# merijn-23/magr-ray-tracer

Measured on AMD Instinct MI355X. Metric: Mrays/sec + extend-kernel HBM GB/s, sponza 1080p 256spp, higher is better.
Workload: dtype f32

## Files before the change

include/rt355.h:

```cpp
#ifndef RT355_H
#define RT355_H
#include "rt355_types.h"

#ifdef __cplusplus
extern "C" {
#endif

#define RT_OK            0
#define RT_E_INVALID    (-1)
#define RT_E_DEVICE     (-2)
#define RT_E_NOMEM      (-3)
#define RT_E_UNSUPPORTED (-4)

#define RT_SHADING_SIMPLE       0
#define RT_SHADING_NEE          1
#define RT_SAMPLING_HEMISPHERE  0
#define RT_SAMPLING_COSINE      1
#define RT_ACCEL_BVH2           0
#define RT_ACCEL_BVH4           1

typedef struct RtCtx RtCtx;

typedef struct RtConfig {
    int32_t width, height;
// ... 12 lines not shown

#define RT_BUILTINS_DEFAULT    0
#define RT_BUILTINS_IEEE       1
#define RT_BUILTINS_REFERENCE  2

typedef struct RtCounters {
    uint64_t extend_rays, extend_tlas_visits, extend_inst_visits, extend_node_visits, extend_prim_tests;
    uint64_t connect_rays, connect_tlas_visits, connect_inst_visits, connect_node_visits, connect_prim_tests;
    uint64_t primary_rays;
    uint64_t shadow_rays;
    uint64_t frames;
    uint64_t extend_node_issues, extend_leaf_issues, connect_node_issues, connect_leaf_issues;
    uint64_t extend_loop_node_events, extend_loop_leaf_events, connect_loop_node_events, connect_loop_leaf_events;
} RtCounters;

typedef struct RtStageTimes {
    double  generate_ms, extend_ms, shade_ms, compact_ms, connect_ms, accumulate_ms;
    int64_t generate_launches, extend_launches, shade_launches, compact_launches, connect_launches, accumulate_launches;
} RtStageTimes;

typedef struct RtKernelInfo {
    int32_t layout;
    int32_t persist, persist4;
    int32_t stack_entries;
    int32_t persist_grid, persist_grid_connect, shade_grid;
    int32_t n_blas;
} RtKernelInfo;

const char* rt_last_error(void);
int rt_device_count(void);
int rt_kernel_info(RtCtx* ctx, RtKernelInfo* out);
int rt_builtins(RtCtx* ctx);
int rt_top_levels(RtCtx* ctx, int32_t* extend, int32_t* connect);

int rt_create(const RtConfig* cfg, RtCtx** out);
int rt_destroy(RtCtx* ctx);

int rt_upload_scene(RtCtx* ctx,
                    const RtPrimitive* prims, int32_t nPrims,
                    const RtMaterial* mats, int32_t nMats,
                    const RtFloat4* textures, int32_t nTexels,
                    const uint32_t* lights, int32_t nLights,
                    const void* bvhNodes, int32_t nNodes,
                    const uint32_t* primIdx, int32_t nIdx,
                    const RtTLASNode* tlas, int32_t nTlas,
                    const RtBVHInstance* blas, int32_t nBlas);

int rt_upload_scene_bvh2(RtCtx* ctx,
                         const RtPrimitive* prims, int32_t nPrims, const RtMaterial* mats, int32_t nMats,
                         const RtFloat4* textures, int32_t nTexels, const uint32_t* lights, int32_t nLights,
                         const RtBVHNode2* bvhNodes, int32_t nNodes, const uint32_t* primIdx, int32_t nIdx,
                         const RtTLASNode* tlas, int32_t nTlas, const RtBVHInstance* blas, int32_t nBlas);

int rt_validate_scene(int32_t accel,
                      const RtPrimitive* prims, int32_t nPrims, const RtMaterial* mats, int32_t nMats,
                      const RtFloat4* textures, int32_t nTexels, const uint32_t* lights, int32_t nLights,
                      const void* bvhNodes, int32_t nNodes, const uint32_t* primIdx, int32_t nIdx,
                      const RtTLASNode* tlas, int32_t nTlas, const RtBVHInstance* blas, int32_t nBlas);

int rt_share_scene(RtCtx* ctx, RtCtx* from);

int rt_build_bvh2(int32_t device, const RtBuildOptions* opts, const RtPrimitive* prims, int32_t nPrims, int32_t first, int32_t count,
                  uint32_t nodeBase, uint32_t idxBase, RtBVHNode2* nodes, int32_t nodeCap, int32_t* nNodes, uint32_t* primIdx,
                  RtBuildStats* stats);
int rt_build_bvh2_sah(int32_t device, const RtPrimitive* prims, int32_t nPrims, int32_t first, int32_t count, uint32_t nodeBase,
                      uint32_t idxBase, RtBVHNode2* nodes, int32_t nodeCap, int32_t* nNodes, uint32_t* primIdx, RtBuildStats* stats);
// ... 141 lines not shown
```

magr_ray_tracer_amd/_lib.py:

```python
import ctypes as C
import os

import numpy as np

_PKG = os.path.dirname(os.path.abspath(__file__))

f4 = np.dtype((np.float32, 4))
Ray = np.dtype([("O", f4), ("D", f4), ("rD", f4), ("N", f4), ("I", f4), ("intensity", f4), ("t", "<f4"),
                ("primIdx", "<i4"), ("bounces", "<i4"), ("pixelIdx", "<i4"), ("inside", "u1"), ("lastSpecular", "u1"),
                ("_pad0", "u1", 2), ("u", "<f4"), ("v", "<f4"), ("_pad1", "<u4")], align=False)
ShadowRay = np.dtype([("I", f4), ("L", f4), ("Nl", f4), ("intensity", f4), ("BRDF", f4), ("lightIdx", "<i4"),
                      ("pixelIdx", "<i4"), ("dotNL", "<f4"), ("dist", "<f4")])
Material = np.dtype([("color", f4), ("absorption", f4), ("specular", "<f4"), ("n1", "<f4"), ("n2", "<f4"),
                     ("isDielectric", "u1"), ("_pad0", "u1", 3), ("texIdx", "<i4"), ("texW", "<i4"), ("texH", "<i4"),
                     ("isLight", "u1"), ("_pad1", "u1", 3), ("emittance", f4)])
Primitive = np.dtype([("v0", f4), ("v1", f4), ("v2", f4), ("N", f4), ("centroid", f4), ("uv0", "<f4", 2), ("uv1", "<f4", 2),
                      ("uv2", "<f4", 2), ("_padt", "<f4", 2), ("objType", "<i4"), ("matIdx", "<i4"), ("area", "<f4"),
                      ("_pad", "<u4")])
Camera = np.dtype([("type", "<i4"), ("fov", "<f4"), ("aperture", "<f4"), ("focalLength", "<f4"), ("forward", f4),
                   ("right", f4), ("up", f4), ("origin", f4), ("horizontal", f4), ("vertical", f4), ("topLeft", f4)])
Settings = np.dtype([("numPrimitives", "<i4"), ("numLights", "<i4"), ("tracerType", "<i4"), ("frames", "<i4"),
                     ("antiAliasing", "<i4"), ("numInRays", "<i4"), ("numOutRays", "<i4"), ("shadowRays", "<i4"),
                     ("renderBVH", "<i4"), ("focalLength", "<f4")])
BVHNode2 = np.dtype([("aabbMin", f4), ("aabbMax", f4), ("first", "<u4"), ("count", "<u4"), ("_pad", "<u4", 2)])
# ... 33 lines not shown
SAMPLING_HEMISPHERE, SAMPLING_COSINE = 0, 1
ACCEL_BVH2, ACCEL_BVH4 = 0, 1
PRIM_SPHERE, PRIM_PLANE, PRIM_TRIANGLE = 0, 1, 2
MATH_EXP, MATH_SIN, MATH_COS, MATH_ACOS, MATH_ATAN, MATH_F2I, MATH_ATAN2, MATH_SPHERE_TEXEL, MATH_NORMALIZE4, MATH_LENGTH4 = range(10)
MATH_WORDS = {MATH_EXP: (1, 1), MATH_SIN: (1, 1), MATH_COS: (1, 1), MATH_ACOS: (1, 1), MATH_ATAN: (1, 1), MATH_F2I: (1, 1),
              MATH_ATAN2: (2, 1), MATH_SPHERE_TEXEL: (6, 2), MATH_NORMALIZE4: (4, 4), MATH_LENGTH4: (4, 1)}
MATH_SWEEP_BLOCK_BITS = 20
MAX_BOUNCES = 7
BUILTINS_DEFAULT, BUILTINS_IEEE, BUILTINS_REFERENCE = 0, 1, 2
BUILTINS = {None: BUILTINS_DEFAULT, "ieee": BUILTINS_IEEE, "reference": BUILTINS_REFERENCE}


def builtins_value(name):
    try:
        return BUILTINS[name]
    except (KeyError, TypeError):
        raise ValueError(f"builtins must be None, 'ieee' or 'reference', not {name!r}") from None


RT_OK, RT_E_INVALID, RT_E_DEVICE, RT_E_NOMEM, RT_E_UNSUPPORTED = 0, -1, -2, -3, -4
SCENE_ARRAYS = {"prims": 0, "bvh": 1, "tlas": 2, "instances": 3, "pairs": 4, "triRecs": 5, "shadeRecs": 6, "lightRecs": 7,
                "tlasPairs": 8, "tlasPairsP": 9, "instRecs": 10}
SCENE_ARRAYS_BVH4 = {"quads": 11, "rootEntry": 12, "bvh2Kept": 13}
UpdateStats = np.dtype([("gpu_ms", "<f8"), ("prims", "<i4"), ("nodes", "<i4"), ("tlas_nodes", "<i4"), ("tlas_depth", "<i4"),
                        ("reconfigured", "<i4"), ("reserved", "<i4", 3)])
assert UpdateStats.itemsize == 40
REBUILD_SAH, REBUILD_LBVH, REBUILD_SBVH = 0, 1, 2
RebuildStats = np.dtype([(n, "<f8") for n in ("gpu_ms", "wall_ms", "stage_ms", "build_ms", "derive_ms", "tlas_ms", "commit_ms")] +
                        [(n, "<i4") for n in ("prims", "blas_built", "nodes", "n_idx", "max_depth", "tlas_nodes", "tlas_depth", "reconfigured")] +
                        [("spatial_splits", "<i4"), ("prims_clipped", "<i4")])
assert RebuildStats.itemsize == 96

DEVICE_SYMBOLS = [
    "rt_last_error", "rt_device_count", "rt_kernel_info", "rt_builtins", "rt_top_levels", "rt_create", "rt_destroy", "rt_upload_scene", "rt_share_scene", "rt_set_seeds", "rt_seed_default",
    "rt_get_seeds", "rt_bind_accum", "rt_accum_device_ptr", "rt_stream", "rt_reset", "rt_render", "rt_synchronize", "rt_focus",
    "rt_read_accum", "rt_write_accum", "rt_postproc", "rt_read_counters", "rt_reset_counters", "rt_read_stage_times", "rt_reset_stage_times", "rt_set_profile",
    "rt_stage_begin_frame", "rt_stage_generate", "rt_stage_extend", "rt_stage_shade", "rt_stage_connect",
    "rt_debug_get_rays", "rt_debug_set_rays", "rt_debug_get_shadow", "rt_debug_enable_steps", "rt_debug_get_steps", "rt_debug_math",
    "rt_debug_math_sweep", "rt_debug_math_mode", "rt_debug_math_sweep_mode", "rt_validate_scene", "rt_build_bvh2", "rt_build_bvh2_sah", "rt_debug_sah_phases", "rt_build_bvh2_sbvh", "rt_debug_sbvh_phases", "rt_update_scene", "rt_group_update_scene", "rt_debug_get_scene_array",
    "rt_rebuild_scene", "rt_group_rebuild_scene", "rt_blas_ranges", "rt_debug_rebuild_allocations",
    "rt_build_bvh4", "rt_upload_scene_bvh2", "rt_group_upload_scene_bvh2",
    "rt_group_create", "rt_group_destroy", "rt_group_lanes", "rt_group_concurrency", "rt_group_lane", "rt_group_frames", "rt_group_upload_scene", "rt_group_share_scene",
    "rt_group_seed", "rt_group_reset", "rt_group_render", "rt_group_synchronize", "rt_group_sum", "rt_group_read_accum", "rt_group_focus",
    "rt_group_postproc"]
HOST_SYMBOLS = [
    "rth_last_error", "rth_scene_create", "rth_scene_destroy", "rth_add_material", "rth_add_texture", "rth_load_texture", "rth_add_sphere",
    "rth_add_plane", "rth_add_triangle", "rth_add_quad", "rth_add_triangles", "rth_build_blas", "rth_build_bvh4",
    "rth_build_tlas", "rth_bvh4_from_nodes", "rth_set_instance_transform", "rth_primitives", "rth_materials", "rth_textures", "rth_lights",
    "rth_bvh2_nodes", "rth_bvh4_nodes", "rth_prim_idx", "rth_tlas_nodes", "rth_blas_nodes", "rth_bvh_stats", "rth_camera",
    "rth_renderer_create", "rth_renderer_destroy", "rth_renderer_init", "rth_renderer_set_camera", "rth_renderer_tick",
    "rth_renderer_read", "rth_renderer_camera", "rth_seed_stream", "rth_load_model", "rth_save_png",
    "rth_set_build_threads", "rth_renderer_save_frame", "rth_renderer_camera_move", "rth_renderer_camera_mouse", "rth_renderer_camera_zoom", "rth_renderer_frames", "rth_renderer_set_lanes", "rth_renderer_set_builtins", "rth_renderer_builtins",
    "rth_build_blas_lbvh", "rth_build_bvh2_lbvh", "rth_lbvh_stats", "rth_set_primitives", "rth_refit",
    "rth_build_blas_sah_gpu", "rth_build_bvh2_sah", "rth_build_blas_sbvh_gpu", "rth_build_bvh2_sbvh", "rth_rebuild", "rth_blas_ranges",
    "rth_build_bvh4_gpu", "rth_build_bvh4_levels"]

_dev = None
_host = None


class NativeLibraryMissing(RuntimeError):
    pass


def _load(name, local=False):
    path = os.path.join(_PKG, name)
    if not os.path.exists(path):
        raise NativeLibraryMissing(
            f"{path} is missing: build it with `python -m magr_ray_tracer_amd.build` (hipcc, gfx950). "
            "The hot path has no Python/CPU fallback.")
    return C.CDLL(path, mode=C.RTLD_LOCAL if local else C.RTLD_GLOBAL)


_variants = {}


def device_lib(variant=None):
    global _dev
    if variant:
        if variant not in _variants:
            keep, _dev = _dev, None
            try:
                _variants[variant] = _bind_device(_load(f"librt355_{variant}.so", local=True))
            finally:
                _dev = keep
        return _variants[variant]
    if _dev is None:
        _dev = _bind_device(_load("librt355.so"))
    return _dev


def _bind_device(lib):
    if True:
        vp, i32, i64 = C.c_void_p, C.c_int32, C.c_int64
        lib.rt_last_error.restype = C.c_char_p
        lib.rt_create.argtypes = [vp, C.POINTER(vp)]
        lib.rt_kernel_info.argtypes = [vp, vp]
        lib.rt_builtins.argtypes = [vp]
        lib.rt_top_levels.argtypes = [vp, C.POINTER(i32), C.POINTER(i32)]
        lib.rt_destroy.argtypes = [vp]
        lib.rt_upload_scene.argtypes = [vp, vp, i32, vp, i32, vp, i32, vp, i32, vp, i32, vp, i32, vp, i32, vp, i32]
        lib.rt_upload_scene_bvh2.argtypes = lib.rt_upload_scene.argtypes
        lib.rt_group_upload_scene_bvh2.argtypes = lib.rt_upload_scene.argtypes
        lib.rt_build_bvh4.argtypes = [i32, vp, i32, i32, vp, i32, vp, vp]
        lib.rt_share_scene.argtypes = [vp, vp]
        lib.rt_set_seeds.argtypes = [vp, vp, i64]
        lib.rt_seed_default.argtypes = [vp]
        lib.rt_get_seeds.argtypes = [vp, vp, i64]
        lib.rt_bind_accum.argtypes = [vp, vp]
        lib.rt_accum_device_ptr.argtypes = [vp]
        lib.rt_accum_device_ptr.restype = vp
        lib.rt_stream.argtypes = [vp]
        lib.rt_stream.restype = vp
        lib.rt_reset.argtypes = [vp]
        lib.rt_render.argtypes = [vp, vp, vp, i32]
        lib.rt_synchronize.argtypes = [vp]
        lib.rt_focus.argtypes = [vp, i32, i32, vp, C.POINTER(C.c_float)]
        lib.rt_read_accum.argtypes = [vp, vp]
        lib.rt_read_counters.argtypes = [vp, vp]
        lib.rt_write_accum.argtypes = [vp, vp]
        lib.rt_postproc.argtypes = [vp, i32, C.c_float, C.c_float, C.c_float, vp, vp]
        lib.rt_reset_counters.argtypes = [vp]
        lib.rt_read_stage_times.argtypes = [vp, vp]
        lib.rt_reset_stage_times.argtypes = [vp]
        lib.rt_set_profile.argtypes = [vp, i32]
        lib.rt_stage_begin_frame.argtypes = [vp]
        lib.rt_stage_generate.argtypes = [vp, vp, vp]
        lib.rt_stage_extend.argtypes = [vp, i32, i32]
        lib.rt_stage_shade.argtypes = [vp, i32]
        lib.rt_stage_connect.argtypes = [vp, i32, i32]
        lib.rt_debug_get_rays.argtypes = [vp, i32, vp, i32, C.POINTER(i32)]
        lib.rt_debug_set_rays.argtypes = [vp, i32, vp, i32]
# ... 120 lines not shown
```

magr_ray_tracer_amd/csrc/rt355.hip:

```cpp
#include <hip/hip_runtime.h>
#include <hip/hip_ext.h>
#include <algorithm>
#include <chrono>
#include <cstdio>
#include <cmath>
#include <cstdlib>
#include <cstring>
#include <memory>
#include <atomic>
#include <string>
#include <vector>
#include "../../include/rt355.h"
#include "rt355_kernels.h"
#include "scene_dev.h"

using namespace rt355dev;
using namespace scenedev;

static constexpr int kAdmitAnySgpr = 6, kAdmit96Sgpr = 7;
static constexpr int kTopLevelsExtend = 6, kTopLevelsConnect = 6;
static constexpr int kFitSeven = 22, kBackupWords = 10, kSpillCap = kFitSeven - kBackupWords;
static thread_local std::string g_err;
int rt355_set_error(int code, const char* msg) { g_err = msg; return code; }

// ... 76 lines not shown
static bool spill_trav(const RtCtx* c) { return c->trav == TRAV_TLAS_SPILL || c->trav == TRAV_BVH4_TLAS_SPILL; }
static bool bvh4_tlas_trav(const RtCtx* c) { return c->trav == TRAV_BVH4_TLAS || c->trav == TRAV_BVH4_TLAS_SPILL; }
static bool tlas_trav(const RtCtx* c) { return c->trav == TRAV_TLAS || c->trav == TRAV_TLAS_SPILL || bvh4_tlas_trav(c); }

extern "C" const char* rt_last_error(void) { return g_err.c_str(); }
extern "C" int rt_device_count(void) { int n = 0; if (hipGetDeviceCount(&n) != hipSuccess) return 0; return n; }
static int sync_scene_config(RtCtx* ctx);
extern "C" int rt_builtins(RtCtx* ctx)
{
    if (!ctx) return fail(RT_E_INVALID, "rt_builtins: null context");
    return ctx->cfg.builtins;
}
extern "C" int rt_kernel_info(RtCtx* ctx, RtKernelInfo* out)
{
    if (!ctx || !out) return fail(RT_E_INVALID, "rt_kernel_info: null argument");
    if (!ctx->sceneLoaded) return fail(RT_E_INVALID, "rt_kernel_info: no scene uploaded");
    if (const int rc = sync_scene_config(ctx)) return rc;
    const int persist = ctx->trav <= TRAV_TLAS_SPILL ? ctx->trav : 0;
    const int persist4 = ctx->trav == TRAV_BVH4 ? 1 : (ctx->trav == TRAV_BVH4_TLAS ? 2 : (ctx->trav == TRAV_BVH4_TLAS_SPILL ? 3 : 0));
    *out = RtKernelInfo{ ctx->layout, persist, persist4, spill_trav(ctx) ? ctx->spillCap : ctx->stackEntries, ctx->persistGrid, ctx->persistGridConnect,
                         ctx->shadeGrid, ctx->sc.nBlas };
    return RT_OK;
}

extern "C" int rt_top_levels(RtCtx* ctx, int32_t* extend, int32_t* connect)
{
    if (!ctx || !extend || !connect) return fail(RT_E_INVALID, "rt_top_levels: null argument");
    if (!ctx->sceneLoaded) return fail(RT_E_INVALID, "rt_top_levels: no scene uploaded");
    if (const int rc = sync_scene_config(ctx)) return rc;
    *extend = ctx->tune.topLevels; *connect = ctx->tuneConnect.topLevels;
    return RT_OK;
}

static void free_bag(std::vector<void*>& bag) { for (void* p : bag) (void)hipFree(p); bag.clear(); }

static void scene_release(RtCtx* ctx)
{
    if (!ctx->scene) return;
    auto& h = ctx->scene->holders;
    h.erase(std::remove(h.begin(), h.end(), ctx), h.end());
    ctx->scene.reset();
}
static void scene_hold(RtCtx* ctx, const std::shared_ptr<SceneBag>& bag)
{
    scene_release(ctx);
    ctx->scene = bag;
    bag->holders.push_back(ctx);
}
int SceneBag::wait_holders() const
{
    for (const RtCtx* h : holders) {
        HIPCHK(hipStreamSynchronize(h->stream));
        if (h->home != h->stream) HIPCHK(hipStreamSynchronize(h->home));
    }
    return RT_OK;
}

static size_t stack_bytes(const RtCtx* c) { return (size_t)c->stackEntries * kBlock * sizeof(uint32_t); }
static size_t top_bytes(int levels) { return levels > 0 ? (((size_t)1 << levels) - 1) * 4 * sizeof(float4) : 0; }
static int tlas_stack_entries(const RtCtx* c) { return c->stackEntries + c->tlasDepth + 1; }
static int tlas_lds_entries(const RtCtx* c) { return spill_trav(c) ? c->spillCap : tlas_stack_entries(c); }
static size_t tlas_column_bytes(int entries) { return (size_t)(entries + kBackupWords) * kBlock * sizeof(uint32_t); }
static size_t tlas_stack_bytes(const RtCtx* c) { return tlas_column_bytes(tlas_lds_entries(c)); }
static inline dim3 grid_for(int n) { return dim3((unsigned)std::max(1, (n + kBlock - 1) / kBlock)); }

using PersistKernel = void (*)(DevScene, DevQueues, int, int, int, PersistTune);
// ... 62 lines not shown
        if (connect) {
            L.tune = c->tuneConnect;
            L.persist = spill ? k_trace_persist4_tlas<true, false, true> : k_trace_persist4_tlas<true>;
            L.grid = dim3(c->persistGridConnect);
            break;
        }
        L.tune = c->tune4;
        if (bounce > 0 || spill) L.grid = dim3(c->persistGrid);
        if (steps) L.persist = spill ? k_trace_persist4_tlas<false, true, true> : k_trace_persist4_tlas<false, true>;
        else L.persist = spill ? k_trace_persist4_tlas<false, false, true> : k_trace_persist4_tlas<false>;
        break;
    }
    }
    return L;
}

static int persist_query(const RtCtx* c, int stage, int topLevels, int* perCU)
{
    const TraceLaunch L = trace_launch(c, stage, stage == ST_CONNECT ? 0 : 1, false, c->nPix, topLevels);
    HIPCHK(hipOccupancyMaxActiveBlocksPerMultiprocessor(perCU, L.persist, kBlock, L.lds));
    return RT_OK;
}
static int persist_blocks(const RtCtx* c, int stage, int perCU, int tuneBlocks)
{
    const bool connect = stage == ST_CONNECT;
    const int fit = std::max(1, perCU);
    int g = std::max(1, std::min(perCU, connect ? kAdmitAnySgpr : kAdmit96Sgpr));
    if (c->cfg.persist_blocks_per_cu > 0) g = std::min(g, std::min(c->cfg.persist_blocks_per_cu, fit));
    if (tuneBlocks > 0) g = std::min(tuneBlocks, fit);
    if (connect) if (const char* t = getenv("RT355_CONNECT_BLOCKS")) { const int d = atoi(t); if (d > 0) g = std::min(d, fit); }
    return g;
}

static constexpr size_t kEvRing = 4096;
static void ev_account(RtCtx* c, RtCtx::Ev& e)
{
    float ms = 0;
    if (hipEventElapsedTime(&ms, e.a, e.b) != hipSuccess) { (void)hipEventSynchronize(e.b); (void)hipEventElapsedTime(&ms, e.a, e.b); }
    switch (e.stage) {
    case ST_GENERATE: c->times.generate_ms += ms; c->times.generate_launches++; break;
    case ST_EXTEND:   c->times.extend_ms += ms; c->times.extend_launches++; break;
    case ST_SHADE:    c->times.shade_ms += ms; c->times.shade_launches++; break;
    case ST_COMPACT:  c->times.compact_ms += ms; c->times.compact_launches++; break;
    case ST_CONNECT:  c->times.connect_ms += ms; c->times.connect_launches++; break;
    case ST_ACCUM:    c->times.accumulate_ms += ms; c->times.accumulate_launches++; break;
    }
    e.stage = -1;
}
static void ev_init(RtCtx* c)
{
    if (!c->cfg.profile || !c->evPool.empty()) return;
    c->evPool.resize(kEvRing);
    for (auto& e : c->evPool) { (void)hipEventCreate(&e.a); (void)hipEventCreate(&e.b); e.stage = -1; }
}
static inline bool ev_on(const RtCtx* c, int stage) { return c->cfg.profile >= 2 || (c->cfg.profile == 1 && stage == ST_EXTEND); }
static void ev_begin(RtCtx* c, int stage)
{
    if (!ev_on(c, stage)) return;
    ev_init(c);
    RtCtx::Ev& e = c->evPool[c->evUsed % kEvRing];
    if (e.stage >= 0) ev_account(c, e);
    e.stage = stage;
    (void)hipEventRecord(e.a, c->stream);
}
static void ev_end(RtCtx* c, int stage)
{
// ... 172 lines not shown
    bool topAuto = false;
    if (ctx->trav == TRAV_BVH2) {
        ctx->tune.topLevels = kTopLevelsExtend; ctx->tuneConnect.topLevels = kTopLevelsConnect;
        topAuto = true;
        if (const char* t = getenv("RT355_TOP_LEVELS")) {
            int a = 0, b = 0;
            const int k = sscanf(t, "%d,%d", &a, &b);
            if (k == 1) b = a;
            if (k >= 1 && a >= 0 && a <= kTopMaxLevels && b >= 0 && b <= kTopMaxLevels) { ctx->tune.topLevels = a; ctx->tuneConnect.topLevels = b; topAuto = false; }
        }
    }
    if (tlas_trav(ctx)) {
        ctx->tune.flat = ctx->tune4.flat = 1; ctx->tuneConnect.flat = 0;
        if (const char* t = getenv("RT355_TLAS_FLAT")) { int a = 0, b = 0; if (sscanf(t, "%d,%d", &a, &b) == 2) { ctx->tune.flat = ctx->tune4.flat = a; ctx->tuneConnect.flat = b; } }
    }
    {
        static std::atomic<int> serial{ 0 };
        if (ctx->xcdFirst < 0) ctx->xcdFirst = serial.fetch_add(1) & 7;
        int rays = 1024;
        if (const char* t = getenv("RT355_XCD_RAYS")) rays = std::max(0, atoi(t));
        ctx->tune.xcdRays = ctx->tuneConnect.xcdRays = ctx->tune4.xcdRays = rays;
        ctx->tune.xcdFirst = ctx->tuneConnect.xcdFirst = ctx->tune4.xcdFirst = ctx->xcdFirst;
        int thin = 16;
        if (const char* t = getenv("RT355_THIN")) thin = std::min(64, std::max(0, atoi(t)));
        ctx->tune.thin = ctx->tuneConnect.thin = ctx->tune4.thin = thin;
    }

    if (persistent(ctx)) {
        int perCU = 0; hipDeviceProp_t prop;
        HIPCHK(hipGetDeviceProperties(&prop, ctx->cfg.device));
        for (PersistTune* t : { &ctx->tune, &ctx->tuneConnect }) if (stack_bytes(ctx) + top_bytes(t->topLevels) > prop.sharedMemPerBlock) t->topLevels = 0;
        if (topAuto) for (int stage : { ST_EXTEND, ST_CONNECT }) {
            PersistTune& t = stage == ST_CONNECT ? ctx->tuneConnect : ctx->tune;
            int q = 0, lv = t.topLevels;
            if (const int rc = persist_query(ctx, stage, 0, &q)) return rc;
            const int base = persist_blocks(ctx, stage, q, tuneBlocks);
            for (; lv > 0; lv--) {
                if (const int rc = persist_query(ctx, stage, lv, &q)) return rc;
                if (persist_blocks(ctx, stage, q, tuneBlocks) == base) break;
            }
            t.topLevels = lv;
        }
        if (const int rc = persist_query(ctx, ST_EXTEND, -1, &perCU)) return rc;
        int perCUc = perCU;
        if (bvh4_tlas_trav(ctx) || ctx->tuneConnect.topLevels > 0) { if (const int rc = persist_query(ctx, ST_CONNECT, -1, &perCUc)) return rc; }
        ctx->persistGrid = std::min(ctx->gridMax, persist_blocks(ctx, ST_EXTEND, perCU, tuneBlocks) * prop.multiProcessorCount);
        ctx->persistGridConnect = std::min(ctx->gridMax, persist_blocks(ctx, ST_CONNECT, perCUc, tuneBlocks) * prop.multiProcessorCount);
    }
    ctx->q.spill = nullptr; ctx->q.spillStride = 0; ctx->q.stackCap = 0;
    ctx->q.tlasLdsEntries = tlas_trav(ctx) ? (uint32_t)tlas_lds_entries(ctx) : 0u;
    if (spill_trav(ctx)) {
        const size_t stride = (size_t)std::max(ctx->persistGrid, ctx->persistGridConnect) * kBlock;
        const size_t words = stride * (size_t)(tlas_stack_entries(ctx) - ctx->spillCap);
        if (words > ctx->spillWords) {
            if (ctx->dSpill) (void)hipFree(ctx->dSpill);
            ctx->dSpill = nullptr; ctx->spillWords = 0;
            if (hipMalloc((void**)&ctx->dSpill, words * sizeof(uint32_t)) != hipSuccess) return fail(RT_E_NOMEM, "hipMalloc of the spill stacks (%zu bytes) failed", words * sizeof(uint32_t));
            ctx->spillWords = words;
        }
        ctx->q.spill = ctx->dSpill; ctx->q.spillStride = (uint32_t)stride; ctx->q.stackCap = (uint32_t)ctx->spillCap;
    }
    return RT_OK;
}

static int adopt_scene(RtCtx* ctx)
{
    const SceneBag& b = *ctx->scene;
    const SceneArrays& a = b.sc;
    auto f4 = [](const RtFloat4* p) { return (const float4*)p; };
    ctx->sc = DevScene{ a.prims, a.mats, f4(a.tex), a.lights, a.bvh2, a.bvh4, a.primIdx, a.tlas, a.blas, f4(a.pairs), f4(a.triRecs), a.rootEntry, f4(a.shadeRecs),
                        f4(a.tlasPairs), f4(a.instRecs), a.tlasRoot, f4(a.tlasPairsP), a.tlasRootP, f4(a.lightRecs), f4(a.quads), a.nLights, a.nPrims, a.nBlas, a.nTex };
    ctx->layout = b.layout; ctx->stackEntries = b.stackEntries; ctx->tlasDepth = b.tlasDepth; ctx->nInterior = b.nInterior; ctx->singleBlas = b.singleBlas;
// ... 909 lines not shown
```

magr_ray_tracer_amd/csrc/rt355_kernels.h:

```cpp
#pragma once
#include <hip/hip_runtime.h>
#include <stdint.h>
#include "../../include/rt355_types.h"

namespace rt355dev {

#define RT_FORCEINLINE __device__ __forceinline__
static constexpr int   kBlock = 256;
static constexpr float kEps = RT_EPSILON;
static constexpr float kFar = RT_REALLYFAR;
static constexpr float kPi = 3.14159274101257f;
static constexpr float kInvPi = 0.31830987334251f;

struct DevScene {
    const RtPrimitive*   prims;
    const RtMaterial*    mats;
    const float4*        tex;
    const uint32_t*      lights;
    const RtBVHNode2*    bvh2;
    const RtBVHNode4*    bvh4;
    const uint32_t*      primIdx;
    const RtTLASNode*    tlas;
    const RtBVHInstance* blas;
    const float4*        pairs;
// ... 1547 lines not shown
{
    ExtRay e;
    e.O = add4(ray.I, muls(T, kEps));
    e.D = T; e.inten = ray.inten; e.bounces = ray.bounces + 1; e.inside = !ray.inside; e.lastSpec = false; e.valid = true;
    return e;
}
template <bool REFB> RT_FORCEINLINE float fresnel(SRay& ray, const RtMaterial* mat, const MatCtl& mc, float4& outT)
{
    float costhetai = dot4(ray.N, muls(ray.D, -1.0f));
    float n1 = mc.n1, n2 = mc.n2;
    if (ray.inside) {
        n1 = mc.n2; n2 = mc.n1;
        ray.inten.x *= rt_expf<REFB>(-mat->absorption.x * ray.t);
        ray.inten.y *= rt_expf<REFB>(-mat->absorption.y * ray.t);
        ray.inten.z *= rt_expf<REFB>(-mat->absorption.z * ray.t);
    }
    float frac = n1 * (1 / n2);
    float k = 1 - frac * frac * (1 - costhetai * costhetai);
    if (k < 0) return 1.f;
    outT = normalize4<REFB>(add4(muls(ray.D, frac), muls(ray.N, frac * costhetai - sqrtf(k))));
    float costhetat = dot4(neg4(ray.N), outT);
    float n1ci = n1 * costhetai, n2ci = n2 * costhetai, n1ct = n1 * costhetat, n2ct = n2 * costhetat;
    float frac1 = (n1ci - n2ct) / (n1ci + n2ct);
    float frac2 = (n1ct - n2ci) / (n1ct + n2ci);
    float Fr = 0.5f * (frac1 * frac1 + frac2 * frac2);
    return mc.specular + (1 - mc.specular) * Fr;
}
template <bool REFB> RT_FORCEINLINE float4 firefly(int on, float4 c)
{
    if (on && dot4(c, c) > 25) return muls(normalize4<REFB>(c), 5.0f);
    return c;
}

struct ShadowOut { float4* a; float4* b; float4* c; bool valid; };

template <bool NEE, bool REFB>
RT_FORCEINLINE float4 shade_hit(const DevScene& sc, const DevVariant& var, SRay& ray, uint32_t& seed, ExtRay& ext, ShadowOut& sh)
{
    const RtPrimitive* prim = sc.prims + ray.prim;
    const RtMaterial* mat = sc.mats + ray.matIdx;
    const MatCtl mc = load_mat_ctl(mat);
    if (mc.isLight) {
        if (NEE && !ray.lastSpec) return splat(0.0f);
        return mul4(ray.inten, ld4(mat->emittance));
    }
    const float rnd = rnd_float(seed);
    if (mc.isDielectric) {
        float4 T = splat(0.0f);
        float Fr = fresnel<REFB>(ray, mat, mc, T);
        ext = rnd < Fr ? reflect_ray(ray) : transmit_ray(ray, T);
        if (NEE) ext.lastSpec = true;
    } else if (rnd < mc.specular) {
        ext = reflect_ray(ray);
        if (NEE) ext.lastSpec = true;
    } else {
        const float4 albedo = albedo_of<REFB>(sc, prim, mat, mc, ray);
        const float4 BRDF = muls(albedo, kInvPi);
        if (NEE && sc.nLights > 0) {
            uint32_t li = f2u_gpu(floorf(rnd_abs(seed) * (float)sc.nLights));
            if (li >= (uint32_t)sc.nLights) li = (uint32_t)sc.nLights - 1;
            const float4* LR = sc.lightRecs + (size_t)li * 8;
            const float4 l0 = LR[0], l1 = LR[1], l2 = LR[2], l3 = LR[3], l4 = LR[4], l5 = LR[5];
            asm volatile("" : : "v"(l0.x), "v"(l1.x), "v"(l2.x), "v"(l3.x), "v"(l4.x), "v"(l5.x));
            const int ltype = __float_as_int(l4.x);
            const float larea = l4.y;
            float4 pl, Nl;
            if (ltype == RT_PRIM_SPHERE) {
                float theta = rnd_abs(seed) * 2.0f * kPi;
                float u = rnd_abs(seed) * 2.0f - 1.0f;
                float pre = sqrtf(1 - u * u);
                float x = rt_cosf<REFB>(theta) * pre, y = rt_sinf<REFB>(theta) * pre;
                pl = add4(muls(mk4(x, y, u, 0.0f), l1.x), l0);
                Nl = muls(sub4(pl, l0), l1.z);
            } else {
                float u1 = rnd_abs(seed), u2 = rnd_abs(seed);
                if (u1 + u2 > 1) { u1 = 1 - u1; u2 = 1 - u2; }
                float4 a = sub4(l1, l0), b = sub4(l2, l0);
                pl = add4(add4(l0, muls(a, u1)), muls(b, u2));
                Nl = ltype == RT_PRIM_PLANE ? l0 : l3;
            }
            float4 dirToLight = sub4(pl, ray.I);
            float dist = length4<REFB>(dirToLight);
            float4 L = muls(dirToLight, 1 / dist);
            float dotNL = dot4(ray.N, L);
            if (dotNL > 0 && dot4(Nl, neg4(L)) > 0) {
                float4 sInt = muls(ray.inten, (float)sc.nLights);
                float solidAngle = dot4(Nl, neg4(L)) * larea * (1 / (dist * dist));
                float4 lightColor = l5;
                float4 Ld = muls(mul4(muls(lightColor, solidAngle), BRDF), dotNL);
                float4 color = firefly<REFB>(var.fireflies, mul4(Ld, sInt));
                float4 so = add4(ray.I, muls(L, kEps));
                *sh.a = mk4(so.x, so.y, so.z, dist - 2 * kEps);
                *sh.b = mk4(L.x, L.y, L.z, __int_as_float(ray.pixel));
                *sh.c = color;
                sh.valid = true;
            }
        }
        if (var.rr) {
            float rr_p = survival_prob(albedo);
            if (rr_p < rnd_float(seed)) return splat(0.0f);
            ray.inten = muls(ray.inten, 1 / rr_p);
        }
        float4 refl = sample_dir<REFB>(var.sampling, ray.N, seed);
        float dotNR = dot4(ray.N, refl);
        float I_PDF = var.sampling == RT_SAMPLING_HEMISPHERE ? 2 * kPi : dotNR * kPi;
        ext.O = add4(ray.I, muls(refl, kEps));
        ext.D = refl;
        if (NEE) ext.inten = muls(muls(mul4(ray.inten, BRDF), I_PDF), dotNR);
        else     ext.inten = mul4(ray.inten, muls(muls(BRDF, I_PDF), dotNR));
        ext.bounces = ray.bounces + 1; ext.inside = ray.inside; ext.lastSpec = false; ext.valid = true;
    }
    return splat(0.0f);
}

static constexpr int kTile = 512;
static constexpr unsigned long long kTileAgg = 1ull << 62, kTilePrefix = 2ull << 62, kTilePrefixZero = 2ull << 62;
RT_FORCEINLINE unsigned long long tile_pack(unsigned long long flag, uint32_t e, uint32_t s) { return flag | ((unsigned long long)e << 31) | (unsigned long long)s; }
RT_FORCEINLINE uint32_t tile_ext(unsigned long long v) { return (uint32_t)((v >> 31) & 0x7fffffffull); }
RT_FORCEINLINE uint32_t tile_sh(unsigned long long v) { return (uint32_t)(v & 0x7fffffffull); }

static constexpr uint32_t kSpinLimit = 1u << 22;
RT_FORCEINLINE unsigned long long wait_word(const unsigned long long* p, unsigned long long needFlag , int32_t* fault, int32_t what = 1)
{
    unsigned long long v = __hip_atomic_load(p, __ATOMIC_RELAXED, __HIP_MEMORY_SCOPE_AGENT);
    uint32_t spins = 0;
    while (needFlag == 2ull ? (v >> 62) != 2ull : (v >> 62) == 0ull) {
        if (++spins > kSpinLimit || ((spins & 1023u) == 0u && __hip_atomic_load(fault, __ATOMIC_RELAXED, __HIP_MEMORY_SCOPE_AGENT) != 0)) { atomicCAS(fault, 0, what); return kTilePrefixZero; }
        if (spins < 4) __builtin_amdgcn_s_sleep(2); else __builtin_amdgcn_s_sleep(32);
        v = __hip_atomic_load(p, __ATOMIC_RELAXED, __HIP_MEMORY_SCOPE_AGENT);
    }
    return v;
}

template <bool NEE, int TILE, bool REFB>
__global__ __launch_bounds__(TILE, 4) void k_shade(DevScene sc, DevQueues q, DevVariant var, int bounce)
{
    __shared__ uint32_t sWaveE[2][TILE / 64], sWaveS[2][TILE / 64], sBaseE, sBaseS;
    __shared__ float4 sExtO[TILE], sExtD[TILE], sExtI[TILE], sShA[2][TILE], sShB[2][TILE], sShC[2][TILE];
    __shared__ uint2 sExtM[TILE];
    const int cur = bounce & 1, nxt = cur ^ 1;
    unsigned long long* state = q.tile[cur];
    unsigned long long* const* super = q.super;
    const int n = q.nRays[bounce];
    if (n <= 0) {
        if (blockIdx.x == 0 && threadIdx.x == 0) { q.nRays[bounce + 1] = 0; q.nShadow[bounce + 1] = q.nShadow[bounce]; }
        return;
    }
    const uint32_t numTiles = (uint32_t)((n + TILE - 1) / TILE);
    const int wave = threadIdx.x >> 6, lane = threadIdx.x & 63;
    const int shadowBase = q.nShadow[bounce];

    auto drain = [&](uint32_t t, int pp, unsigned long long em, unsigned long long sm, bool extValid, bool shValid) {
        if (wave == 0) {
            uint32_t aggE = 0, aggS = 0;
#pragma unroll
            for (int w = 0; w < TILE / 64; w++) { aggE += sWaveE[pp][w]; aggS += sWaveS[pp][w]; }
            const uint32_t sup = t >> 6, inSup = t & 63u;
            unsigned long long v = 0ull;
            if ((uint32_t)lane < inSup) v = wait_word(&state[1 + (sup << 6) + (uint32_t)lane], 0ull, q.fault, 0x10000000 | (int32_t)((sup << 6) + (uint32_t)lane));
            else if (lane == 63 && sup > 0) v = wait_word(&super[cur][sup - 1], 2ull, q.fault, 0x20000000 | (int32_t)(sup - 1));
            const unsigned long long vp = __shfl(v, 63, 64);
            const uint32_t preE = sup > 0 ? tile_ext(vp) : 0u, preS = sup > 0 ? tile_sh(vp) : 0u;
            uint32_t inE = (uint32_t)lane < inSup ? tile_ext(v) : 0u, inS = (uint32_t)lane < inSup ? tile_sh(v) : 0u;
#pragma unroll
            for (int off = 32; off > 0; off >>= 1) { inE += __shfl_xor(inE, off, 64); inS += __shfl_xor(inS, off, 64); }
            if (lane == 0) {
                sBaseE = preE + inE; sBaseS = preS + inS;
                if (t == numTiles - 1) { q.nRays[bounce + 1] = (int)(preE + inE + aggE); q.nShadow[bounce + 1] = shadowBase + (int)(preS + inS + aggS); }
            }
        }
        __syncthreads();
        uint32_t baseE = sBaseE, baseS = sBaseS + (uint32_t)shadowBase;
        for (int w = 0; w < wave; w++) { baseE += sWaveE[pp][w]; baseS += sWaveS[pp][w]; }
        const unsigned long long below = (1ull << lane) - 1ull;
        if (extValid) {
            const uint32_t dst = baseE + (uint32_t)__popcll(em & below);
            q.O[nxt][dst] = sExtO[threadIdx.x]; q.D[nxt][dst] = sExtD[threadIdx.x]; q.inten[nxt][dst] = sExtI[threadIdx.x];
            q.meta[nxt][dst] = sExtM[threadIdx.x];
        }
        if (shValid) {
            const uint32_t dst = baseS + (uint32_t)__popcll(sm & below);
            q.sA[dst] = sShA[pp][threadIdx.x]; q.sB[dst] = sShB[pp][threadIdx.x]; q.sC[dst] = sShC[pp][threadIdx.x];
        }
        __syncthreads();
    };

#ifdef RT355_SHADE_TIMING
    long long tShade = 0, tDrain = 0, tBegin = wall_clock64(); int nT = 0;
#endif
    bool pend = false, pExt = false, pSh = false;
    uint32_t pTile = 0;
    unsigned long long pEm = 0ull, pSm = 0ull;
    int par = 0;
    struct TileIn { float4 hit, O, D, inten; uint2 meta; uint32_t seed; };
    auto fetch = [&](uint32_t t, TileIn& in) {
        const int j = (int)t * TILE + threadIdx.x;
        if (t < numTiles && j < n) {
            in.hit = ldnt4(&q.hit[j]); in.meta = ldnt2(&q.meta[cur][j]); in.O = ldnt4(&q.O[cur][j]); in.D = ldnt4(&q.D[cur][j]); in.inten = ldnt4(&q.inten[cur][j]);
            in.seed = q.seeds[j];
        }
    };
    __shared__ uint32_t sTicket;
    const uint32_t cls = blockIdx.x % (uint32_t)kTicketClasses;
    int32_t* ticket = q.shadeTicket + ((size_t)bounce * kTicketClasses + cls) * kTicketStride;
    uint32_t tkNext = 0;
    if (threadIdx.x == 0) sTicket = (uint32_t)atomicAdd(ticket, 1);
    __syncthreads();
    uint32_t tile = sTicket * (uint32_t)kTicketClasses + cls;
    __syncthreads();
    TileIn in;
    fetch(tile, in);
    for (; tile < numTiles; par ^= 1) {
        const int i = (int)tile * TILE + threadIdx.x;
        if (threadIdx.x == 0) {
            q.tile[nxt][1 + tile] = 0ull;
            tkNext = (uint32_t)atomicAdd(ticket, 1);
        }
#ifdef RT355_SHADE_TIMING
        const long long c0 = wall_clock64();
#endif

        bool extValid = false, shValid = false;
        ExtRay ext; ext.valid = false;
        uint2 extMeta = make_uint2(0u, 0u);
        if (i < n) {
            ShadowOut sh; sh.valid = false; sh.a = &sShA[par][threadIdx.x]; sh.b = &sShB[par][threadIdx.x]; sh.c = &sShC[par][threadIdx.x];
            const float4 hit = in.hit;
            const uint2 meta = in.meta;
            SRay ray;
            ray.O = in.O; ray.D = in.D; ray.inten = in.inten;
            ray.t = hit.x; ray.prim = __float_as_int(hit.y); ray.u = hit.z; ray.v = hit.w;
            ray.pixel = (int)meta.x; ray.bounces = (int)(meta.y & kMetaBounceMask);
            ray.inside = (meta.y & kMetaInside) != 0; ray.lastSpec = (meta.y & kMetaLastSpec) != 0;
            if (ray.prim == -1) {
                float4 c = mul4(ray.inten, mk4(0.0784f, 0.0941f, 0.3215f, 0.0f));
                q.accum[ray.pixel] = add4(q.accum[ray.pixel], c);
            } else {
                ray.I = add4(ray.O, muls(ray.D, ray.t));
                const float4 rec = sc.shadeRecs[ray.prim];
                asm volatile("" : : "v"(rec.x), "v"(rec.w));
                const uint32_t tag = __float_as_uint(rec.w);
                ray.matIdx = (int)(tag & 0x07ffffffu);
                ray.N = (tag >> 28) == RT_PRIM_SPHERE ? prim_normal(sc.prims + ray.prim, ray.I)
                                                      : mk4(rec.x, rec.y, rec.z, (tag & 0x08000000u) ? -0.0f : 0.0f);
                if (dot4(ray.N, neg4(ray.D)) < 0) ray.N = muls(ray.N, -1.0f);
                uint32_t seed = in.seed;
                float4 color = shade_hit<NEE, REFB>(sc, var, ray, seed, ext, sh);
                q.seeds[i] = seed;
                color = firefly<REFB>(var.fireflies, color);
                if (color.x != 0.0f || color.y != 0.0f || color.z != 0.0f || color.w != 0.0f)
                    q.accum[ray.pixel] = add4(q.accum[ray.pixel], color);
                if (ext.valid && ext.bounces <= RT_MAX_BOUNCES) {
                    extValid = true;
                    extMeta = make_uint2((uint32_t)ray.pixel, (uint32_t)ext.bounces | (ext.inside ? kMetaInside : 0u) | (ext.lastSpec ? kMetaLastSpec : 0u));
                }
                shValid = sh.valid;
            }
        }
        const unsigned long long em = __ballot(extValid), sm = __ballot(shValid);
// ... 18 lines not shown
                uint32_t preE = 0, preS = 0;
                if (sup > 0) {
                    if (lane == 0) __hip_atomic_store(&super[cur][sup], tile_pack(kTileAgg, totE, totS), __ATOMIC_RELAXED, __HIP_MEMORY_SCOPE_AGENT);
                    int top = (int)sup - 1;
                    for (;;) {
                        const int tt = top - lane;
                        unsigned long long v = kTilePrefix;
                        if (tt >= 0) v = wait_word(&super[cur][tt], 0ull, q.fault, 0x30000000 | tt);
                        const unsigned long long isPre = __ballot((v >> 62) == 2ull);
                        const int stop = isPre ? __ffsll((long long)isPre) - 1 : 64;
                        uint32_t e = lane <= stop ? tile_ext(v) : 0u, s2 = lane <= stop ? tile_sh(v) : 0u;
#pragma unroll
                        for (int off = 32; off > 0; off >>= 1) { e += __shfl_xor(e, off, 64); s2 += __shfl_xor(s2, off, 64); }
                        preE += e; preS += s2;
                        if (isPre) break;
                        top -= 64;
                    }
                }
                if (lane == 0) __hip_atomic_store(&super[cur][sup], tile_pack(kTilePrefix, preE + totE, preS + totS), __ATOMIC_RELAXED, __HIP_MEMORY_SCOPE_AGENT);
            }
        }
#ifdef RT355_SHADE_TIMING
        const long long c1 = wall_clock64();
#endif
        const uint32_t nextTile = sTicket * (uint32_t)kTicketClasses + cls;
        TileIn inNext;
        fetch(nextTile, inNext);
        if (pend) drain(pTile, par ^ 1, pEm, pSm, pExt, pSh);
        else __syncthreads();
        in = inNext;
#ifdef RT355_SHADE_TIMING
        tShade += c1 - c0; tDrain += wall_clock64() - c1; nT++;
#endif
        if (extValid) { sExtO[threadIdx.x] = ext.O; sExtD[threadIdx.x] = ext.D; sExtI[threadIdx.x] = ext.inten; sExtM[threadIdx.x] = extMeta; }
        pend = true; pTile = tile; pEm = em; pSm = sm; pExt = extValid; pSh = shValid;
        tile = nextTile;
    }
    if (pend) {
        __syncthreads();
        drain(pTile, par ^ 1, pEm, pSm, pExt, pSh);
    }
#ifdef RT355_SHADE_TIMING
    if (threadIdx.x == 0 && (blockIdx.x & 127) == 5 && bounce <= 1)
        printf("shade b%d block %d tiles %d: shade %lld drain %lld total %lld (x10 ns)\n", bounce, blockIdx.x, nT, tShade, tDrain, wall_clock64() - tBegin);
#endif
}

template <int ACCEL, int LAYOUT>
__global__ __launch_bounds__(kBlock) void k_connect(DevScene sc, DevQueues q, int b0, int b1)
{
    extern __shared__ uint32_t stk[];
    const int first = q.nShadow[b0], n = q.nShadow[b1 + 1] - first;
    const int i = blockIdx.x * kBlock + threadIdx.x;
    WorkCtr wc = { 0, 0, 0, 0 };
    uint32_t rays = 0;
    if (i < n) {
        const float4 a = q.sA[first + i], b = q.sB[first + i];
        TRay r;
        r.ox = a.x; r.oy = a.y; r.oz = a.z; r.dx = b.x; r.dy = b.y; r.dz = b.z;
        r.rx = 1.0f / b.x; r.ry = 1.0f / b.y; r.rz = 1.0f / b.z;
        r.t = a.w; r.prim = -1; r.u = 0.0f; r.v = 0.0f;
        rays = 1;
        if (traverse_tlas<ACCEL, LAYOUT, true>(sc, r, stk, wc) == -1) q.sC[first + i] = splat(0.0f);
    }
    flush_counters(q.ctrConnect, rays, wc, stk);
}

// ... 101 lines not shown
```

magr_ray_tracer_amd/renderer.py:

```python
import ctypes as C

import numpy as np

from . import _lib


class RtError(RuntimeError):
    code = None


def _update_args(prims, first, instances):
    p = None if prims is None else np.ascontiguousarray(prims, dtype=_lib.Primitive)
    b = None if instances is None else np.ascontiguousarray(instances, dtype=_lib.BVHInstance)
    st = np.zeros((), dtype=_lib.UpdateStats)
    args = (_lib.ptr(p) if p is not None and len(p) else None, int(first), 0 if p is None else len(p),
            _lib.ptr(b) if b is not None else None, 0 if b is None else len(b), _lib.ptr(st))
    return args, (p, b), st


def _update_dict(st):
    return {"gpu_ms": float(st["gpu_ms"]), "prims": int(st["prims"]), "nodes": int(st["nodes"]), "tlas_nodes": int(st["tlas_nodes"]),
            "tlas_depth": int(st["tlas_depth"]), "reconfigured": bool(st["reconfigured"])}


# ... 92 lines not shown
    def rebuild_scene(self, prims=None, first=0, instances=None, builder="sah", alpha=None, **lbvh_options):
        args, keep, st = _rebuild_args(prims, first, instances, builder, lbvh_options, alpha)
        rc = self._lib.rt_rebuild_scene(self._h, *args)
        if rc != 0:
            e = RtError(self._lib.rt_last_error().decode())
            e.code = rc
            raise e
        return _rebuild_dict(st)

    def rebuild_allocations(self):
        n = C.c_int64(0)
        self._chk(self._lib.rt_debug_rebuild_allocations(self._h, C.byref(n)))
        return n.value

    def scene_array(self, name):
        which = _lib.SCENE_ARRAYS[name] if name in _lib.SCENE_ARRAYS else _lib.SCENE_ARRAYS_BVH4[name]
        n = C.c_int64(0)
        self._chk(self._lib.rt_debug_get_scene_array(self._h, which, None, 0, C.byref(n)))
        out = np.zeros(n.value, dtype=np.uint8)
        if n.value:
            self._chk(self._lib.rt_debug_get_scene_array(self._h, which, _lib.ptr(out), n.value, C.byref(n)))
        return out

    def kernel_info(self):
        k = np.zeros((), dtype=_lib.KernelInfo)
        self._chk(self._lib.rt_kernel_info(self._h, k.ctypes.data_as(C.c_void_p)))
        return {n: int(k[n]) for n in k.dtype.names}

    def top_levels(self):
        e, c = C.c_int32(0), C.c_int32(0)
        self._chk(self._lib.rt_top_levels(self._h, C.byref(e), C.byref(c)))
        return int(e.value), int(c.value)

    @property
    def builtins(self):
        rc = self._lib.rt_builtins(self._h)
        if rc < 0:
            self._chk(rc)
        return int(rc)

    def extend_kernel_name(self):
        k = self.kernel_info()
        if k["persist4"] == 3:
            return "k_trace_persist4_tlas<false, false, true> (LDS stack of %d entries per lane, deeper entries in global memory)" % k["stack_entries"]
        if k["persist4"] == 2:
            return "k_trace_persist4_tlas<false> (bounce 0: its one-ray-per-lane branch)"
        if k["persist4"]:
            return "k_trace_persist4<false>"
        if k["persist"] == 3:
            return "k_trace_persist_tlas<false, false, true> (LDS stack of %d entries per lane, deeper entries in global memory)" % k["stack_entries"]
        if k["persist"] == 2:
            return "k_trace_persist_tlas<false> (bounce 0: its one-ray-per-lane branch)"
        if k["persist"]:
            return "k_trace_persist<false> (bounce 0: <false, true>, node records of wave-uniform visits through the scalar cache)"
        return "k_extend<%s, %d>" % ("RT_ACCEL_BVH4" if self.accel == _lib.ACCEL_BVH4 else "RT_ACCEL_BVH2", k["layout"])

    def set_seeds(self, seeds):
        s = np.ascontiguousarray(seeds, dtype=np.uint32)
        self._chk(self._lib.rt_set_seeds(self._h, _lib.ptr(s), s.size))

    def seed_default(self):
        self._chk(self._lib.rt_seed_default(self._h))

    def get_seeds(self):
        s = np.zeros(self.npix, dtype=np.uint32)
        self._chk(self._lib.rt_get_seeds(self._h, _lib.ptr(s), s.size))
# ... 305 lines not shown
```

Measured before the change: 1011.

## Shrink shade kernel LDS parking and size top-level cache around co-resident shade

The shade kernel's shared-memory staging for extension and shadow rays is repacked. The double-buffered shadow arrays become single-buffered, shadow direction is stored as float2, pixel and z are shared in one array, and ray meta is packed into one byte. Shadow outputs are kept in registers instead of written through LDS pointers. Separately, when persistent traversal blocks share CUs with shade, the top-level LDS cache depth is chosen so that as many traversal blocks still fit beside the shade kernel, estimated from LDS, VGPR and wave-slot counts. A footprint query API is added. The smaller LDS footprint is meant to raise occupancy and co-residency, at the cost of more live registers and changed drain ordering.

```diff
diff --git a/include/rt355.h b/include/rt355.h
--- a/include/rt355.h
+++ b/include/rt355.h
@@ -68,6 +68,7 @@
 int rt_kernel_info(RtCtx* ctx, RtKernelInfo* out);
 int rt_builtins(RtCtx* ctx);
 int rt_top_levels(RtCtx* ctx, int32_t* extend, int32_t* connect);
+int rt_shade_footprint(RtCtx* ctx, int32_t* ldsBytes, int32_t* traversalBeside);
 
 int rt_create(const RtConfig* cfg, RtCtx** out);
 int rt_destroy(RtCtx* ctx);
diff --git a/magr_ray_tracer_amd/_lib.py b/magr_ray_tracer_amd/_lib.py
--- a/magr_ray_tracer_amd/_lib.py
+++ b/magr_ray_tracer_amd/_lib.py
@@ -89,7 +89,7 @@
 assert RebuildStats.itemsize == 96
 
 DEVICE_SYMBOLS = [
-    "rt_last_error", "rt_device_count", "rt_kernel_info", "rt_builtins", "rt_top_levels", "rt_create", "rt_destroy", "rt_upload_scene", "rt_share_scene", "rt_set_seeds", "rt_seed_default",
+    "rt_last_error", "rt_device_count", "rt_kernel_info", "rt_builtins", "rt_top_levels", "rt_shade_footprint", "rt_create", "rt_destroy", "rt_upload_scene", "rt_share_scene", "rt_set_seeds", "rt_seed_default",
     "rt_get_seeds", "rt_bind_accum", "rt_accum_device_ptr", "rt_stream", "rt_reset", "rt_render", "rt_synchronize", "rt_focus",
     "rt_read_accum", "rt_write_accum", "rt_postproc", "rt_read_counters", "rt_reset_counters", "rt_read_stage_times", "rt_reset_stage_times", "rt_set_profile",
     "rt_stage_begin_frame", "rt_stage_generate", "rt_stage_extend", "rt_stage_shade", "rt_stage_connect",
@@ -155,6 +155,7 @@
         lib.rt_kernel_info.argtypes = [vp, vp]
         lib.rt_builtins.argtypes = [vp]
         lib.rt_top_levels.argtypes = [vp, C.POINTER(i32), C.POINTER(i32)]
+        lib.rt_shade_footprint.argtypes = [vp, C.POINTER(i32), C.POINTER(i32)]
         lib.rt_destroy.argtypes = [vp]
         lib.rt_upload_scene.argtypes = [vp, vp, i32, vp, i32, vp, i32, vp, i32, vp, i32, vp, i32, vp, i32, vp, i32]
         lib.rt_upload_scene_bvh2.argtypes = lib.rt_upload_scene.argtypes
diff --git a/magr_ray_tracer_amd/csrc/rt355.hip b/magr_ray_tracer_amd/csrc/rt355.hip
--- a/magr_ray_tracer_amd/csrc/rt355.hip
+++ b/magr_ray_tracer_amd/csrc/rt355.hip
@@ -132,6 +132,25 @@
     return RT_OK;
 }
 
+static int beside_shade(const RtCtx* c, int stage, int topLevels, int* perCU, int* shadeLds);
+extern "C" int rt_shade_footprint(RtCtx* ctx, int32_t* ldsBytes, int32_t* traversalBeside)
+{
+    if (!ctx || !ldsBytes || !traversalBeside) return fail(RT_E_INVALID, "rt_shade_footprint: null argument");
+    if (!ctx->sceneLoaded) return fail(RT_E_INVALID, "rt_shade_footprint: no scene uploaded");
+    if (const int rc = sync_scene_config(ctx)) return rc;
+    *ldsBytes = 0; *traversalBeside = 0;
+    if (!persistent(ctx)) {
+        hipFuncAttributes a{};
+        HIPCHK(hipFuncGetAttributes(&a, (const void*)ctx->kShade));
+        *ldsBytes = (int32_t)a.sharedSizeBytes;
+        return RT_OK;
+    }
+    int lds = 0, beside = 0;
+    if (const int rc = beside_shade(ctx, ST_EXTEND, 0, &beside, &lds)) return rc;
+    *ldsBytes = lds; *traversalBeside = beside;
+    return RT_OK;
+}
+
 static void free_bag(std::vector<void*>& bag) { for (void* p : bag) (void)hipFree(p); bag.clear(); }
 
 static void scene_release(RtCtx* ctx)
@@ -260,6 +279,28 @@
     return g;
 }
 
+static constexpr size_t kLdsBlock = 1280;
+static int beside_shade(const RtCtx* c, int stage, int topLevels, int* perCU, int* shadeLds)
+{
+    const TraceLaunch L = trace_launch(c, stage, stage == ST_CONNECT ? 0 : 1, false, c->nPix, topLevels);
+    hipFuncAttributes shade{}, trav{};
+    hipDeviceProp_t prop;
+    HIPCHK(hipGetDeviceProperties(&prop, c->cfg.device));
+    HIPCHK(hipFuncGetAttributes(&shade, (const void*)c->kShade));
+    HIPCHK(hipFuncGetAttributes(&trav, (const void*)L.persist));
+    auto alloc = [](int regs) { return std::max(8, (regs + 7) / 8 * 8); };
+    const size_t ldsCU = std::max(prop.maxSharedMemoryPerMultiProcessor, prop.sharedMemPerBlock);
+    auto blocks = [](size_t bytes) { return (bytes + kLdsBlock - 1) / kLdsBlock * kLdsBlock; };
+    const size_t travLds = blocks(trav.sharedSizeBytes + L.lds), shadeLdsCU = blocks(shade.sharedSizeBytes);
+    const int shadeWaves = std::max(1, c->shadeTile / kBlock);
+    const int byLds = ldsCU > shadeLdsCU && travLds > 0 ? (int)((ldsCU - shadeLdsCU) / travLds) : 0;
+    const int byVgpr = (512 - shadeWaves * alloc(shade.numRegs)) / alloc(trav.numRegs);
+    const int bySlots = 8 - shadeWaves;
+    *perCU = std::max(0, std::min(std::min(byLds, byVgpr), std::min(bySlots, stage == ST_CONNECT ? kAdmitAnySgpr : kAdmit96Sgpr)));
+    *shadeLds = (int)shade.sharedSizeBytes;
+    return RT_OK;
+}
+
 static constexpr size_t kEvRing = 4096;
 static void ev_account(RtCtx* c, RtCtx::Ev& e)
 {
@@ -498,12 +539,18 @@
         for (PersistTune* t : { &ctx->tune, &ctx->tuneConnect }) if (stack_bytes(ctx) + top_bytes(t->topLevels) > prop.sharedMemPerBlock) t->topLevels = 0;
         if (topAuto) for (int stage : { ST_EXTEND, ST_CONNECT }) {
             PersistTune& t = stage == ST_CONNECT ? ctx->tuneConnect : ctx->tune;
-            int q = 0, lv = t.topLevels;
+            int q = 0, lv = t.topLevels, beside = 0, shadeLds = 0;
+            const bool shared = ctx->cfg.persist_blocks_per_cu > 0;
             if (const int rc = persist_query(ctx, stage, 0, &q)) return rc;
             const int base = persist_blocks(ctx, stage, q, tuneBlocks);
+            if (shared) { if (const int rc = beside_shade(ctx, stage, 0, &beside, &shadeLds)) return rc; }
             for (; lv > 0; lv--) {
                 if (const int rc = persist_query(ctx, stage, lv, &q)) return rc;
-                if (persist_blocks(ctx, stage, q, tuneBlocks) == base) break;
+                if (persist_blocks(ctx, stage, q, tuneBlocks) != base) continue;
+                if (!shared) break;
+                int fit = 0;
+                if (const int rc = beside_shade(ctx, stage, lv, &fit, &shadeLds)) return rc;
+                if (fit >= beside) break;
             }
             t.topLevels = lv;
         }
diff --git a/magr_ray_tracer_amd/csrc/rt355_kernels.h b/magr_ray_tracer_amd/csrc/rt355_kernels.h
--- a/magr_ray_tracer_amd/csrc/rt355_kernels.h
+++ b/magr_ray_tracer_amd/csrc/rt355_kernels.h
@@ -1603,7 +1603,7 @@
     return c;
 }
 
-struct ShadowOut { float4* a; float4* b; float4* c; bool valid; };
+struct ShadowOut { float4 a, b, c; bool valid; };
 
 template <bool NEE, bool REFB>
 RT_FORCEINLINE float4 shade_hit(const DevScene& sc, const DevVariant& var, SRay& ray, uint32_t& seed, ExtRay& ext, ShadowOut& sh)
@@ -1661,9 +1661,9 @@
                 float4 Ld = muls(mul4(muls(lightColor, solidAngle), BRDF), dotNL);
                 float4 color = firefly<REFB>(var.fireflies, mul4(Ld, sInt));
                 float4 so = add4(ray.I, muls(L, kEps));
-                *sh.a = mk4(so.x, so.y, so.z, dist - 2 * kEps);
-                *sh.b = mk4(L.x, L.y, L.z, __int_as_float(ray.pixel));
-                *sh.c = color;
+                sh.a = mk4(so.x, so.y, so.z, dist - 2 * kEps);
+                sh.b = mk4(L.x, L.y, L.z, __int_as_float(ray.pixel));
+                sh.c = color;
                 sh.valid = true;
             }
         }
@@ -1703,12 +1703,19 @@
     return v;
 }
 
+static_assert(RT_MAX_BOUNCES < 0x40 && kMetaInside == 0x100u && kMetaLastSpec == 0x200u, "park_meta packs meta.y into one byte");
+RT_FORCEINLINE uint8_t park_meta(uint32_t y) { return (uint8_t)((y & 0x3fu) | ((y & (kMetaInside | kMetaLastSpec)) >> 2)); }
+RT_FORCEINLINE uint32_t unpark_meta(uint8_t b) { return ((uint32_t)b & 0x3fu) | (((uint32_t)b & 0xc0u) << 2); }
 template <bool NEE, int TILE, bool REFB>
 __global__ __launch_bounds__(TILE, 4) void k_shade(DevScene sc, DevQueues q, DevVariant var, int bounce)
 {
     __shared__ uint32_t sWaveE[2][TILE / 64], sWaveS[2][TILE / 64], sBaseE, sBaseS;
-    __shared__ float4 sExtO[TILE], sExtD[TILE], sExtI[TILE], sShA[2][TILE], sShB[2][TILE], sShC[2][TILE];
-    __shared__ uint2 sExtM[TILE];
+    enum { P_EXT_O, P_EXT_D, P_EXT_I, P_SH_A, P_SH_C, P_ROWS4 = NEE ? 5 : 3 };
+    __shared__ float4 sPark4[P_ROWS4 * TILE];
+    __shared__ float2 sShB[NEE ? TILE : 1];
+    __shared__ uint2 sPixZ[TILE];
+    __shared__ uint8_t sExtM[TILE];
+    auto park_slot = [] { uint32_t s = threadIdx.x; asm volatile("" : "+v"(s)); return s; };
     const int cur = bounce & 1, nxt = cur ^ 1;
     unsigned long long* state = q.tile[cur];
     unsigned long long* const* super = q.super;
@@ -1744,14 +1751,16 @@
         uint32_t baseE = sBaseE, baseS = sBaseS + (uint32_t)shadowBase;
         for (int w = 0; w < wave; w++) { baseE += sWaveE[pp][w]; baseS += sWaveS[pp][w]; }
         const unsigned long long below = (1ull << lane) - 1ull;
+        const uint32_t slot = park_slot();
         if (extValid) {
             const uint32_t dst = baseE + (uint32_t)__popcll(em & below);
-            q.O[nxt][dst] = sExtO[threadIdx.x]; q.D[nxt][dst] = sExtD[threadIdx.x]; q.inten[nxt][dst] = sExtI[threadIdx.x];
-            q.meta[nxt][dst] = sExtM[threadIdx.x];
-        }
-        if (shValid) {
+            q.O[nxt][dst] = sPark4[P_EXT_O * TILE + slot]; q.D[nxt][dst] = sPark4[P_EXT_D * TILE + slot]; q.inten[nxt][dst] = sPark4[P_EXT_I * TILE + slot];
+            q.meta[nxt][dst] = make_uint2(sPixZ[slot].x, unpark_meta(sExtM[slot]));
+        }
+        if (NEE && shValid) {
             const uint32_t dst = baseS + (uint32_t)__popcll(sm & below);
-            q.sA[dst] = sShA[pp][threadIdx.x]; q.sB[dst] = sShB[pp][threadIdx.x]; q.sC[dst] = sShC[pp][threadIdx.x];
+            const float2 bxy = sShB[slot]; const uint2 pz = sPixZ[slot];
+            q.sA[dst] = sPark4[P_SH_A * TILE + slot]; q.sB[dst] = mk4(bxy.x, bxy.y, __uint_as_float(pz.y), __uint_as_float(pz.x)); q.sC[dst] = sPark4[P_SH_C * TILE + slot];
         }
         __syncthreads();
     };
@@ -1793,9 +1802,9 @@
 
         bool extValid = false, shValid = false;
         ExtRay ext; ext.valid = false;
+        ShadowOut sh; sh.valid = false;
         uint2 extMeta = make_uint2(0u, 0u);
         if (i < n) {
-            ShadowOut sh; sh.valid = false; sh.a = &sShA[par][threadIdx.x]; sh.b = &sShB[par][threadIdx.x]; sh.c = &sShC[par][threadIdx.x];
             const float4 hit = in.hit;
             const uint2 meta = in.meta;
             SRay ray;
@@ -1880,7 +1889,10 @@
 #ifdef RT355_SHADE_TIMING
         tShade += c1 - c0; tDrain += wall_clock64() - c1; nT++;
 #endif
-        if (extValid) { sExtO[threadIdx.x] = ext.O; sExtD[threadIdx.x] = ext.D; sExtI[threadIdx.x] = ext.inten; sExtM[threadIdx.x] = extMeta; }
+        const uint32_t slot = park_slot();
+        if (extValid) { sPark4[P_EXT_O * TILE + slot] = ext.O; sPark4[P_EXT_D * TILE + slot] = ext.D; sPark4[P_EXT_I * TILE + slot] = ext.inten; sExtM[slot] = park_meta(extMeta.y); }
+        if (NEE && shValid) { sPark4[P_SH_A * TILE + slot] = sh.a; sShB[slot] = make_float2(sh.b.x, sh.b.y); sPark4[P_SH_C * TILE + slot] = sh.c; }
+        if (extValid || shValid) sPixZ[slot] = make_uint2(shValid ? __float_as_uint(sh.b.w) : extMeta.x, __float_as_uint(sh.b.z));
         pend = true; pTile = tile; pEm = em; pSm = sm; pExt = extValid; pSh = shValid;
         tile = nextTile;
     }
diff --git a/magr_ray_tracer_amd/renderer.py b/magr_ray_tracer_amd/renderer.py
--- a/magr_ray_tracer_amd/renderer.py
+++ b/magr_ray_tracer_amd/renderer.py
@@ -148,6 +148,11 @@
         self._chk(self._lib.rt_top_levels(self._h, C.byref(e), C.byref(c)))
         return int(e.value), int(c.value)
 
+    def shade_footprint(self):
+        b, t = C.c_int32(0), C.c_int32(0)
+        self._chk(self._lib.rt_shade_footprint(self._h, C.byref(b), C.byref(t)))
+        return int(b.value), int(t.value)
+
     @property
     def builtins(self):
         rc = self._lib.rt_builtins(self._h)
```

Result: faster. 1022 (median of 6 runs) (+1.1%).
